# fallenshock/SinDDM

Hardware: AMD Instinct MI355X
Metric: diffusion steps/sec (finest scale) + imgs/sec full multi-scale sample, 1/2/4/8 GPU (higher is better)
Workload: dtype f32 (3x3 convs: binary16 hi/lo split products -- Winograd-domain GEMMs with all 4 MFMA terms, fp32 accumulate; fp32-equivalent, error vs float64 = the fp32 oracle's: tests/test_gpu_h2.py; everything else fp32); 1 GPU; C3: 6-scale pyramid, T=1000, finest scale 411x512, batch 64 per GPU, dim=160; batch_per_gpu=64, global_batch=64, scale=5, parallelism=independent chains over 1 GPU(s), one all-gather of the images

## Files before the change

### sinddm_amd/csrc/conv_wh.h

```cpp
#pragma once
#include <utility>
#include "split16.h"

namespace sinddm {

template <class F, int... I>
__device__ __forceinline__ void wh_static_for_impl(F&& f, std::integer_sequence<int, I...>) {
    (f(std::integral_constant<int, I>{}), ...);
}
template <int N, class F>
__device__ __forceinline__ void wh_static_for(F&& f) {
    wh_static_for_impl(f, std::make_integer_sequence<int, N>{});
}

#ifndef WH_ABL
#define WH_ABL 0
#endif
#ifndef WH_MIXLO
#define WH_MIXLO 1
#endif
#ifndef WH_NT
#define WH_NT 6
#endif
#ifdef WH_TIMING
__device__ unsigned long long g_wh_seg[8 * 256 * 8 * 32];
#define WH_SEG(slot) do { if (j == 2) g_wh_seg[((p.mtp * 256 + blockIdx.x) * 8 + wv) * 32 + (slot)] = __builtin_amdgcn_s_memtime(); } while (0)
#else
#define WH_SEG(slot) do {} while (0)
#endif
constexpr int WH_TH = 8, WH_TW = 32;
constexpr int WH_RS = 40;
constexpr int WH_PS = 408;
constexpr int WH_RAW = 16 * WH_PS * 4;
constexpr int WH_V = 24 * 2 * 64 * 16;
constexpr int WH_XS = 36;
constexpr int WH_X = 2 * 6 * 32 * WH_XS * 4;
constexpr int WH_LDS = 160 * 1024;
constexpr int WH_REGION = WH_LDS - WH_RAW;
constexpr int WH_VB = WH_REGION - WH_V;
static_assert(WH_X <= WH_VB && WH_V + WH_X <= WH_REGION && WH_VB % 16 == 0, "exchange buffer beside either V buffer");
constexpr int WH_TARGET_EXP = 10;
constexpr int WH_COB = 80;

inline bool wh_shape_ok(int cin, int cout) { return cin >= 32 && cin % 16 == 0 && cout % WH_COB == 0; }
inline long long wh_image_halfs(int cin, int cout) { return (long long)(cout / WH_COB) * (cin / 16) * 24 * 5 * 512; }

__device__ __forceinline__ int wh_shift_for(float m, int target) {
    const unsigned bits = __float_as_uint(m) & 0x7fffffffu;
    const int e = (int)(bits >> 23);
    if (e == 0 || e == 255) return 0;
    int s = target - (e - 127);
    return s > 100 ? 100 : (s < -100 ? -100 : s);
}

__device__ __forceinline__ void wh_u24(const float* __restrict__ w, long long base, int transpose, double (&u)[24]) {
    const double G2[4][3] = {{1., 0., 0.}, {.5, .5, .5}, {.5, -.5, .5}, {0., 0., 1.}};
    const double G4[6][3] = {{1. / 4, 0., 0.}, {-1. / 6, -1. / 6, -1. / 6}, {-1. / 6, 1. / 6, -1. / 6},
                             {1. / 24, 1. / 12, 1. / 6}, {1. / 24, -1. / 12, 1. / 6}, {0., 0., 1.}};
    double g[3][3];
#pragma unroll
    for (int a = 0; a < 3; ++a)
#pragma unroll
        for (int b = 0; b < 3; ++b) g[a][b] = (double)(transpose ? w[base + (2 - a) * 3 + (2 - b)] : w[base + a * 3 + b]);
#pragma unroll
    for (int i = 0; i < 4; ++i)
#pragma unroll
        for (int j = 0; j < 6; ++j) {
            double acc = 0.;
#pragma unroll
            for (int a = 0; a < 3; ++a) {
                double r = 0.;
#pragma unroll
                for (int b = 0; b < 3; ++b) r += G4[j][b] * g[a][b];
                acc += G2[i][a] * r;
            }
            u[i * 6 + j] = acc;
        }
}

__global__ __launch_bounds__(256) void wh_wscale_kernel(const float* __restrict__ w, float* __restrict__ wsinv, int cin,
                                                         int cout, int transpose) {
    const int m = blockIdx.x;
    const int M = transpose ? cin : cout, K = transpose ? cout : cin;
    float mx = 0.f;
    if (m < M)
        for (int k = threadIdx.x; k < K; k += 256) {
            double u[24];
            wh_u24(w, transpose ? ((long long)k * cin + m) * 9 : ((long long)m * cin + k) * 9, transpose, u);
#pragma unroll
            for (int f = 0; f < 24; ++f) mx = fmaxf(mx, fabsf((float)u[f]));
        }
    __shared__ float red[4];
#pragma unroll
    for (int o = 32; o > 0; o >>= 1) mx = fmaxf(mx, __shfl_xor(mx, o));
    if ((threadIdx.x & 63) == 0) red[threadIdx.x >> 6] = mx;
    __syncthreads();
    if (threadIdx.x == 0 && m < M) {
        mx = fmaxf(fmaxf(red[0], red[1]), fmaxf(red[2], red[3]));
        wsinv[m] = h2_pow2(-h2_shift_for(mx));
    }
}

__global__ __launch_bounds__(256) void wh_pack_kernel(const float* __restrict__ w, const float* __restrict__ wsinv,
                                                       _Float16* __restrict__ img, int cin, int cout, int transpose,
                                                       long long total) {
    const long long i = (long long)blockIdx.x * 256 + threadIdx.x;
    if (i >= total) return;
    const int M = transpose ? cin : cout, K = transpose ? cout : cin;
    const int nch = K / 16;
    long long r = i;
    const int e = (int)(r % 8); r /= 8;
    const int co16 = (int)(r % 16); r /= 16;
    const int kh = (int)(r % 2); r /= 2;
    const int n = (int)(r % 5); r /= 5;
    const int ch = (int)(r % nch); r /= nch;
    const int cb = (int)r;
    const int m = cb * WH_COB + n * 16 + co16;
    const int k = ch * 16 + kh * 8 + e;
    double u[24];
    if (m < M && k < K) wh_u24(w, transpose ? ((long long)k * cin + m) * 9 : ((long long)m * cin + k) * 9, transpose, u);
    else {
#pragma unroll
        for (int f = 0; f < 24; ++f) u[f] = 0.;
    }
    const double sc = m < M ? 1.0 / (double)wsinv[m] : 1.0;
#pragma unroll
    for (int f = 0; f < 24; ++f) {
        const double s = u[f] * sc;
        const _Float16 hi = (_Float16)(float)s;
        const _Float16 lo = (_Float16)(float)(s - (double)(float)hi);
        const long long o = ((((long long)(cb * nch + ch) * 24 + f) * 5 + n) * 2) * 256 + (kh * 16 + co16) * 8 + e;
        img[o] = hi;
        img[o + 256] = lo;
    }
}

inline int wh_pack_launch(const float* w, float* wsinv, void* img, int cin, int cout, int transpose, hipStream_t st) {
    const int M = transpose ? cin : cout, K = transpose ? cout : cin;
    hipLaunchKernelGGL(wh_wscale_kernel, dim3(M), dim3(256), 0, st, w, wsinv, cin, cout, transpose);
    SINDDM_LAUNCH_CHECK();
    const long long total = (long long)(M / WH_COB) * (K / 16) * 5 * 2 * 16 * 8;
    hipLaunchKernelGGL(wh_pack_kernel, dim3((unsigned)((total + 255) / 256)), dim3(256), 0, st, w, wsinv,
                       static_cast<_Float16*>(img), cin, cout, transpose, total);
    SINDDM_LAUNCH_CHECK();
    return 0;
}

__device__ __forceinline__ void wh_barrier() { asm volatile("s_waitcnt lgkmcnt(0)\n\ts_barrier" ::: "memory"); }

__device__ __forceinline__ float wh_dpp_shr2(float old, float src) {
    return __builtin_bit_cast(float, __builtin_amdgcn_update_dpp(__builtin_bit_cast(int, old), __builtin_bit_cast(int, src), 0x112, 0xf, 0xf, false));
}
__device__ __forceinline__ float wh_dpp_shl2(float old, float src) {
    return __builtin_bit_cast(float, __builtin_amdgcn_update_dpp(__builtin_bit_cast(int, old), __builtin_bit_cast(int, src), 0x102, 0xf, 0xf, false));
}

__global__ __launch_bounds__(512) void conv_wh_kernel(ConvArgs p, int items_per_xcd, int wg_per_xcd) {
    typedef __attribute__((address_space(3))) float lds_f;
    extern __shared__ __attribute__((aligned(16))) float smem[];
    unsigned char* const sbytes = reinterpret_cast<unsigned char*>(smem);
    unsigned char* const sRaw = sbytes;
    unsigned char* const sV = sbytes + WH_RAW;
    const unsigned lds0 = (unsigned)(size_t)(lds_f*)smem;

    const int tid = threadIdx.x;
    const int lane = tid & 63;
    const int wv = __builtin_amdgcn_readfirstlane(tid >> 6);
    const int l16 = lane & 15, kq = lane >> 4;
    const int H = p.H, W = p.W;
    const int HW = H * W;
    const int Wt = p.Wt > 0 ? p.Wt : W;
    const int nch = p.nch3;
    const bool big_out = __builtin_amdgcn_readfirstlane((size_t)p.B * p.Cout * HW > ((size_t)1 << 28)) != 0;
    constexpr int OOB = 0x40000000;
    const bool service_rt = wv >= 6;
    const int sv = wv - 6;

    const int t_q = lane & 1, t_tc = (lane >> 1) & 7, t_mg = (lane >> 4) & 1, t_trl = lane >> 5;
    const int t_tr = t_mg * 2 + t_trl, t_t16 = t_trl * 8 + t_tc;
    const int t_rdB = (((sv & 1) * 8 + 4 * t_q) * WH_PS + 2 * t_tr * WH_RS + 4 * t_tc + 4) * 4;
    const int t_rdE = (((sv & 1) * 8 + 4 * t_q) * WH_PS + 2 * t_tr * WH_RS + (t_tc == 7 ? 36 : 3)) * 4;
    const int t_wr0 = ((t_mg * 64 + (sv & 1) * 16 + t_t16) * 16) + t_q * 8;
    const int fj = service_rt ? 0 : wv;
    const int a_rd = ((kq & 1) * 16 + l16) * 16;

    const int xcd = blockIdx.x & 7, ls = blockIdx.x >> 3;
    const int tpi = p.tilesX * p.tilesY;
    struct Item { int b, y0, x0, cb; bool ok; };
    auto decode = [&](int j) {
        Item it;
        const int li = ls + j * wg_per_xcd;
        const int tl = li / p.coblks;
        it.cb = li - tl * p.coblks;
        const int tile = xcd * p.tiles_per_xcd + tl;
        it.ok = li < items_per_xcd && tile < p.ntiles;
        const int tcl = it.ok ? tile : 0;
        it.b = tcl / tpi;
        const int trm = tcl - it.b * tpi;
        const int tyi = trm / p.tilesX;
        it.y0 = tyi * WH_TH;
        it.x0 = (trm - tyi * p.tilesX) * WH_TW;
        return it;
    };
    auto stage_offsets = [&](const Item& it, int (&vo)[2]) {
#pragma unroll
        for (int ps = 0; ps < 2; ++ps) {
            const int qd = ps * 64 + lane;
            const int r = qd / 10, g = qd - r * 10;
            const int gy = it.y0 - 1 + r, gx = it.x0 - 4 + 4 * g;
            vo[ps] = (qd < 100 && gy >= 0 && gy < H && gx >= 0 && gx < W) ? (gy * W + gx) * 4 : OOB;
        }
    };
    auto role_body = [&](auto ROLE) {
    constexpr bool service = decltype(ROLE)::value;
    f32x4 stg[16];
    auto stage_load = [&](const __amdgpu_buffer_rsrc_t& rs, const int (&vo)[2], int c) {
#pragma unroll
        for (int k = 0; k < 8; ++k) {
            const int so = (c * 16 + (sv & 1) * 8 + k) * HW * 4;
            stg[2 * k] = (WH_ABL & 1) ? f32x4{0.f, 0.f, 0.f, 0.f} : __builtin_bit_cast(f32x4, __builtin_amdgcn_raw_buffer_load_b128(rs, vo[0], so, (WH_NT & 1) ? 2 : 0));
            stg[2 * k + 1] = (WH_ABL & 1) ? f32x4{0.f, 0.f, 0.f, 0.f} : __builtin_bit_cast(f32x4, __builtin_amdgcn_raw_buffer_load_b128(rs, vo[1], so, (WH_NT & 1) ? 2 : 0));
        }
    };
    auto stage_write = [&](unsigned char* raw) {
        unsigned char* dst = raw + (sv & 1) * 8 * WH_PS * 4 + lane * 16;
#pragma unroll
        for (int k = 0; k < 8; ++k) {
            *reinterpret_cast<f32x4*>(dst + k * WH_PS * 4) = stg[2 * k];
            if (lane < 36) *reinterpret_cast<f32x4*>(dst + k * WH_PS * 4 + 1024) = stg[2 * k + 1];
        }
    };
    auto in_rsrc = [&](int b) {
        return __builtin_amdgcn_make_buffer_rsrc(const_cast<float*>(p.in + (size_t)b * p.Cin * HW), 0, p.Cin * HW * 4, 0x00020000);
    };

    Item cur = decode(0);
    if (!cur.ok) return;
    int svoff[2] = {OOB, OOB};
#ifndef WH_SVC_PRIO
#define WH_SVC_PRIO 2
#endif
    if constexpr (service) __builtin_amdgcn_s_setprio(WH_SVC_PRIO);
    if constexpr (service) {
        stage_offsets(cur, svoff);
        stage_load(in_rsrc(cur.b), svoff, 0);
    }
    auto item_scale = [&](const Item& it, float& sxo, float& inv) {
        const int xs = p.amax_in ? wh_shift_for(p.amax_in[(size_t)it.b * AMAX_STRIDE], WH_TARGET_EXP) : 0;
        const float sg = (((it.x0 >> 5) + (it.y0 >> 3) + it.b) & 1) ? -1.0f : 1.0f;
        sxo = sg * h2_pow2(xs);
        inv = sg * h2_pow2(-xs);
    };
    int g = 0;
    auto vbuf = [&](int k) { return sV + ((k & 1) ? WH_VB : 0); };
    for (int j = 0;; ++j) {
        const Item nxt = decode(j + 1);
        const int cb = cur.cb, b = cur.b, y0 = cur.y0, x0 = cur.x0;
        float sx, inv_sx;
        item_scale(cur, sx, inv_sx);

        const __amdgpu_buffer_rsrc_t rsin = in_rsrc(b);

        auto transform = [&](const unsigned char* raw, unsigned char* vb, float sxv) {
            if (WH_ABL & 2) return;
            const f32x2 sx2{sxv, sxv};
            const unsigned char* rpB = raw + t_rdB;
            const unsigned char* rpE = raw + t_rdE;
            unsigned char* wp = vb + t_wr0;
            f32x2 d[2][4][6];
#pragma unroll
            for (int pr = 0; pr < 2; ++pr)
#pragma unroll
                for (int rr = 0; rr < 4; ++rr) {
                    const int o = ((2 * pr) * WH_PS + rr * WH_RS) * 4;
                    const f32x4 a4 = *reinterpret_cast<const f32x4*>(rpB + o), b4 = *reinterpret_cast<const f32x4*>(rpB + o + WH_PS * 4);
                    const float ae = *reinterpret_cast<const float*>(rpE + o), be = *reinterpret_cast<const float*>(rpE + o + WH_PS * 4);
                    d[pr][rr][0] = f32x2{wh_dpp_shr2(ae, a4[3]), wh_dpp_shr2(be, b4[3])};
                    d[pr][rr][1] = f32x2{a4[0], b4[0]}; d[pr][rr][2] = f32x2{a4[1], b4[1]};
                    d[pr][rr][3] = f32x2{a4[2], b4[2]}; d[pr][rr][4] = f32x2{a4[3], b4[3]};
                    d[pr][rr][5] = f32x2{wh_dpp_shl2(ae, a4[0]), wh_dpp_shl2(be, b4[0])};
                }
            wh_static_for<4>([&](auto II) {
                constexpr int i = decltype(II)::value;
                h16x2 hi[2][6], lo[2][6];
#pragma unroll
                for (int pr = 0; pr < 2; ++pr) {
                    f32x2 r[6];
#pragma unroll
                    for (int c = 0; c < 6; ++c)
                        r[c] = i == 0 ? d[pr][0][c] - d[pr][2][c] : i == 1 ? d[pr][1][c] + d[pr][2][c]
                             : i == 2 ? d[pr][2][c] - d[pr][1][c] : d[pr][1][c] - d[pr][3][c];
                    const f32x2 s24 = r[4] - 4.f * r[2], s13 = r[3] - 4.f * r[1];
                    const f32x2 u24 = r[4] - r[2], d31 = r[3] - r[1];
                    f32x2 v[6];
                    v[0] = 4.f * r[0] + (r[4] - 5.f * r[2]);
                    v[1] = s24 + s13;
                    v[2] = s24 - s13;
                    v[3] = u24 + 2.f * d31;
                    v[4] = u24 - 2.f * d31;
                    v[5] = 4.f * r[1] + (r[5] - 5.f * r[3]);
#pragma unroll
                    for (int j = 0; j < 6; ++j) {
                        const f32x2 sc = v[j] * sx2;
                        hi[pr][j] = __builtin_convertvector(sc, h16x2);
#if WH_MIXLO
                        lo[pr][j] = h16x2{(_Float16)__builtin_fmaf(v[j].x, sxv, -(float)hi[pr][j].x), (_Float16)__builtin_fmaf(v[j].y, sxv, -(float)hi[pr][j].y)};
#else
                        const f32x2 rem{__builtin_fmaf(v[j].x, sxv, -(float)hi[pr][j].x), __builtin_fmaf(v[j].y, sxv, -(float)hi[pr][j].y)};
                        lo[pr][j] = __builtin_convertvector(rem, h16x2);
#endif
                    }
                }
#pragma unroll
                for (int j = 0; j < 6; ++j) {
                    using h16x4 = __attribute__((ext_vector_type(4))) _Float16;
                    *reinterpret_cast<h16x4*>(wp + (i * 6 + j) * 2048) = h16x4{hi[0][j][0], hi[0][j][1], hi[1][j][0], hi[1][j][1]};
                    *reinterpret_cast<h16x4*>(wp + (i * 6 + j) * 2048 + 512) = h16x4{lo[0][j][0], lo[0][j][1], lo[1][j][0], lo[1][j][1]};
                }
            });
        };

        f32x4 acc[4][2][5];
#pragma unroll
        for (int a = 0; a < 4; ++a)
#pragma unroll
            for (int g = 0; g < 2; ++g)
#pragma unroll
                for (int n = 0; n < 5; ++n) acc[a][g][n] = f32x4{0.f, 0.f, 0.f, 0.f};
        const __amdgpu_buffer_rsrc_t rsw =
            __builtin_amdgcn_make_buffer_rsrc(const_cast<float*>(p.w3), 0, 0x7FFFFFF0, 0x00020000);
        const int wlane = lane * 16;
        const int wbase = ((cb * nch) * 24 + fj) * 5 * 1024;
        h16x8 ur[10];
        auto load_u = [&](int c, int fi, int n, int slot) {
            const int so = wbase + (c * 24 * 5 + fi * 30 + n) * 1024;
            ur[slot] = __builtin_bit_cast(h16x8, __builtin_amdgcn_raw_buffer_load_b128(rsw, wlane, so, 0));
        };
        auto multiply = [&](int c, const unsigned char* vb) {
            const unsigned char* A = vb + fj * 2048 + a_rd;
            wh_static_for<4>([&](auto FI) {
                constexpr int fi = decltype(FI)::value;
                constexpr int fo = fi * 6 * 2048;
                h16x8 ah0, ah1, al0, al1;
                ah0 = *reinterpret_cast<const h16x8*>(A + fo);
                ah1 = *reinterpret_cast<const h16x8*>(A + fo + 1024);
                al0 = *reinterpret_cast<const h16x8*>(A + fo + 512);
                al1 = *reinterpret_cast<const h16x8*>(A + fo + 1024 + 512);
                wh_static_for<5>([&](auto NN) {
                    constexpr int n = decltype(NN)::value;
                    constexpr int slot = (fi & 1) * 5 + n;
                    const h16x8 u = ur[slot];
                    __builtin_amdgcn_sched_barrier(0);
                    if (WH_ABL & 8) {
                        asm volatile("" ::"v"(ah0), "v"(ah1), "v"(al0), "v"(al1), "v"(u));
                    } else {
                        acc[fi][0][n] = __builtin_amdgcn_mfma_f32_16x16x32_f16(al0, u, acc[fi][0][n], 0, 0, 0);
                        acc[fi][1][n] = __builtin_amdgcn_mfma_f32_16x16x32_f16(al1, u, acc[fi][1][n], 0, 0, 0);
                        acc[fi][0][n] = __builtin_amdgcn_mfma_f32_16x16x32_f16(ah0, u, acc[fi][0][n], 0, 0, 0);
                        acc[fi][1][n] = __builtin_amdgcn_mfma_f32_16x16x32_f16(ah1, u, acc[fi][1][n], 0, 0, 0);
                    }
                    __builtin_amdgcn_sched_barrier(0);
                    if (!(WH_ABL & 4)) {
                        if (fi < 2) load_u(c, fi + 2, n, slot);
                        else load_u(c + 1 < nch ? c + 1 : c, fi - 2, n, slot);
                    }
                    __builtin_amdgcn_sched_barrier(0);
                });
            });
        };

        const int e_t = tid & 31, e_co = tid >> 5;
        const int e_tr = e_t >> 3, e_tc = e_t & 7;
        const int ey = y0 + 2 * e_tr, ex = x0 + 4 * e_tc;
        f32x4 rsd[5][2];
        float ek[5], ebv[5];
        auto ep_operands = [&]() {
            const bool e_in = ex < W;
#pragma unroll
            for (int n = 0; n < 5; ++n) {
                const int co = cb * WH_COB + n * 16 + e_co;
                ek[n] = inv_sx * p.wsinv[co];
                ebv[n] = p.bias ? p.bias[co] : 0.0f;
#pragma unroll
                for (int pp = 0; pp < 2; ++pp) {
                    rsd[n][pp] = f32x4{0.f, 0.f, 0.f, 0.f};
                    if (p.resid && !(WH_ABL & 16) && e_in && ey + pp < H)
                        rsd[n][pp] = ((WH_NT & 2) && big_out) ? __builtin_nontemporal_load(reinterpret_cast<const f32x4*>(p.resid + ((size_t)b * p.Cout + co) * HW + (size_t)(ey + pp) * W + ex))
                                                 : *reinterpret_cast<const f32x4*>(p.resid + ((size_t)b * p.Cout + co) * HW + (size_t)(ey + pp) * W + ex);
                }
            }
        };

        WH_SEG(0);
        if constexpr (service) {
            const __amdgpu_buffer_rsrc_t rsnx = in_rsrc(nxt.ok ? nxt.b : b);
            float sxn = 0.f, inv_n = 0.f;
            if (nxt.ok) item_scale(nxt, sxn, inv_n);
            if (j == 0) {
                stage_write(sRaw);
                if (nch > 1) stage_load(rsin, svoff, 1);
                else if (nxt.ok) { stage_offsets(nxt, svoff); stage_load(rsnx, svoff, 0); }
                WH_SEG(1);
                transform(sRaw, vbuf(g), sx);
                wh_barrier();
            }
            WH_SEG(2);
            for (int c = 0; c < nch; ++c) {
                if (c + 1 < nch || nxt.ok) {
                    stage_write(sRaw);
                    if (c + 2 < nch) stage_load(rsin, svoff, c + 2);
                    else if (nxt.ok) {
                        if (c + 2 == nch) stage_offsets(nxt, svoff);
                        if (c + 2 == nch || nch > 1) stage_load(rsnx, svoff, c + 2 - nch);
                    }
                    if (c == 3) WH_SEG(24);
                    transform(sRaw, vbuf(g + c + 1), c + 1 < nch ? sx : sxn);
                    if (c == 3) WH_SEG(25);
                }
                wh_barrier();
                if (c < 12) WH_SEG(3 + c);
            }
            ep_operands();
        } else {
            wh_static_for<10>([&](auto SL) {
                constexpr int sl = decltype(SL)::value;
                load_u(0, sl / 5, sl % 5, sl);
            });
            WH_SEG(1);
            if (j == 0) wh_barrier();
            WH_SEG(2);
            for (int c = 0; c < nch; ++c) {
                multiply(c, vbuf(g + c));
                if (c == 3) WH_SEG(25);
                wh_barrier();
                if (c < 12) WH_SEG(3 + c);
            }
            ep_operands();
        }
        g += nch;
        WH_SEG(16);

        const int e_wr = ((fj * 32 + l16) * WH_XS + 4 * kq) * 4;
        const int e_rd = (e_co * WH_XS + e_t) * 4;
        float amax = 0.f;
        WH_SEG(17);
        if constexpr (!service) {
#pragma unroll
            for (int mg = 0; mg < 2; ++mg)
#pragma unroll
                for (int n = 0; n < 5; ++n) {
                    acc[0][mg][n] = acc[0][mg][n] + acc[1][mg][n] + acc[2][mg][n];
                    acc[1][mg][n] = acc[1][mg][n] - acc[2][mg][n] - acc[3][mg][n];
                }
        }
        wh_static_for<3>([&](auto PS) {
            constexpr int n0 = 2 * decltype(PS)::value;
            constexpr int nn = n0 + 2 <= 5 ? 2 : 1;
            unsigned char* X = sV + ((g & 1) ? 0 : WH_V);
            if constexpr (!service) {
#pragma unroll
                for (int r = 0; r < 2; ++r)
#pragma unroll
                    for (int nl = 0; nl < nn; ++nl)
#pragma unroll
                        for (int mg = 0; mg < 2; ++mg)
                            *reinterpret_cast<f32x4*>(X + e_wr + (r * 6 * 32 + nl * 16) * (WH_XS * 4) + mg * 64) = acc[r][mg][n0 + nl];
            }
            wh_barrier();
            WH_SEG(18 + decltype(PS)::value);
            float q[nn][2][6];
#pragma unroll
            for (int nl = 0; nl < nn; ++nl)
#pragma unroll
                for (int r = 0; r < 2; ++r)
#pragma unroll
                    for (int j = 0; j < 6; ++j)
                        q[nl][r][j] = *reinterpret_cast<const float*>(X + e_rd + ((r * 6 + j) * 32 + nl * 16) * (WH_XS * 4));
            wh_barrier();
            wh_static_for<nn>([&](auto NL) {
                constexpr int n = n0 + decltype(NL)::value;
                const int co = cb * WH_COB + n * 16 + e_co;
                const float k = ek[n];
                const float bv = ebv[n];
#pragma unroll
                for (int pp = 0; pp < 2; ++pp) {
                    const float* z = q[decltype(NL)::value][pp];
                    const float s12 = z[1] + z[2], d12 = z[1] - z[2], s34 = z[3] + z[4], d34 = z[3] - z[4];
                    f32x4 v{z[0] + s12 + s34, d12 + 2.f * d34, s12 + 4.f * s34, d12 + 8.f * d34 + z[5]};
                    const int y = ey + pp;
                    if ((WH_ABL & 16) && v[0] != 123.456f) continue;
                    if (y < H && ex < W) {
                        const size_t o = ((size_t)b * p.Cout + co) * HW + (size_t)y * W + ex;
                        v = v * k + bv;
                        if (p.out_pre) *reinterpret_cast<f32x4*>(p.out_pre + o) = v;
                        if (p.act == 1) v = gelu_erf4(v);
                        else if (p.act == 2) {
                            const f32x4 a = *reinterpret_cast<const f32x4*>(p.aux + o);
#pragma unroll
                            for (int e = 0; e < 4; ++e) v[e] *= gelu_erf_grad(a[e]);
                        }
                        v += rsd[n][pp];
                        if (ex + 4 > Wt) {
#pragma unroll
                            for (int e = 0; e < 4; ++e) v[e] = ex + e < Wt ? v[e] : 0.0f;
                        }
#pragma unroll
                        for (int e = 0; e < 4; ++e) amax = fmaxf(amax, fabsf(v[e]));
                        if ((WH_NT & 4) && big_out) __builtin_nontemporal_store(v, reinterpret_cast<f32x4*>(p.out + o));
                        else *reinterpret_cast<f32x4*>(p.out + o) = v;
                    }
                }
            });
        });
        if (p.amax_out) amax_publish(amax, p.amax_out + (size_t)b * AMAX_STRIDE);
        WH_SEG(23);
        if (!nxt.ok) break;
        cur = nxt;
    }
    };
    if (service_rt) role_body(std::true_type{});
    else role_body(std::false_type{});
}

#ifndef SINDDM_WH_MIN_ITEMS_PER_CU
#define SINDDM_WH_MIN_ITEMS_PER_CU 12
#endif
#ifndef SINDDM_WH_MIN_PIXELS
#define SINDDM_WH_MIN_PIXELS 12000
#endif
#ifndef SINDDM_CONV_WH
#define SINDDM_CONV_WH 1
#endif
inline bool conv_wh_applies(bool fp32_convs, int B, int H, int W, int cin, int cout) {
    if (!SINDDM_CONV_WH || fp32_convs || !wh_shape_ok(cin, cout) || W % 4 != 0) return false;
    if ((long long)cin * H * W * 4 >= 0x40000000LL) return false;
    if ((long long)H * W < SINDDM_WH_MIN_PIXELS) return false;
    return (long long)B * ((W + WH_TW - 1) / WH_TW) * ((H + WH_TH - 1) / WH_TH) * (cout / WH_COB) >=
           (long long)SINDDM_WH_MIN_ITEMS_PER_CU * wino2_cu_count();
}

inline int conv_wh_launch(const ConvArgs& a_in, hipStream_t st) {
    ConvArgs a = a_in;
    if (!wh_shape_ok(a.Cin, a.Cout) || a.W % 4 != 0 || !a.wsinv || (long long)a.Cin * a.H * a.W * 4 >= 0x40000000LL)
        return SINDDM_E_BADSHAPE;
    ConvProfiler& prof = conv_profiler();
    const bool rec = prof.on && prof.used < ConvProfiler::MAXREC;
    if (rec) {
        while (prof.created <= prof.used) {
            (void)hipEventCreate(&prof.ev[2 * prof.created]);
            (void)hipEventCreate(&prof.ev[2 * prof.created + 1]);
            ++prof.created;
        }
        (void)hipEventRecord(prof.ev[2 * prof.used], st);
    }
    a.nch3 = a.Cin / 16;
    a.coblks = a.Cout / WH_COB;
    a.tilesX = (a.W + WH_TW - 1) / WH_TW;
    a.tilesY = (a.H + WH_TH - 1) / WH_TH;
    a.ntiles = a.B * a.tilesX * a.tilesY;
    a.tiles_per_xcd = (a.ntiles + 7) / 8;
    const int ipx = a.tiles_per_xcd * a.coblks;
    int wpx = wino2_cu_count() / 8;
    if (wpx < 1) wpx = 1;
    if (wpx > ipx) wpx = ipx;
    static const hipError_t attr_rc = hipFuncSetAttribute(reinterpret_cast<const void*>(&conv_wh_kernel),
                                                          hipFuncAttributeMaxDynamicSharedMemorySize, WH_LDS);
    if (attr_rc != hipSuccess) return (int)attr_rc;
#ifdef WH_TIMING
    static int wh_launch_no = 0;
    a.mtp = wh_launch_no++ % 8;
#endif
    hipLaunchKernelGGL(conv_wh_kernel, dim3(wpx * 8), dim3(512), WH_LDS, st, a, ipx, wpx);
    if (rec) {
        (void)hipEventRecord(prof.ev[2 * prof.used + 1], st);
        const double fl = 2.0 * a.B * a.H * (a.Wt > 0 ? a.Wt : a.W) * (double)a.Cout * 9.0 * a.Cin;
        prof.note(1, fl, 2.0 * a.ntiles * 32.0 * 24.0 * 4.0 * (double)a.Cout * a.Cin, 8);
    }
    SINDDM_LAUNCH_CHECK();
    return 0;
}

}
```

### sinddm_amd/csrc/plan.h

```cpp
#pragma once
#include <stdint.h>

namespace sinddm {

constexpr int KC = 8;
constexpr int TIME_DIM = 32;
constexpr int CHANNELS = 3;

inline bool wh_plan_ok(int cin, int cout) { return cin >= 32 && cin % 16 == 0 && cout % 80 == 0; }
inline long long wh_plan_halfs(int cin, int cout) { return (long long)(cout / 80) * (cin / 16) * 24 * 5 * 512; }

struct BlockPlan {
    int cin, cout;
    int64_t mlp_w, mlp_b, tr_w, tr_b, dw_w, dw_b, c1_w, c1_b, c2_w, c2_b, res_w, res_b;
    int mt;
    int coblks;
    int co_lds;
    int nch1;
    int nch2;
    int nchr;
    int64_t pk_c1, pk_c2, pk_res, pk_b1, pk_b2;
    int nchw1, nchw2;
    int64_t pk_wc1, pk_wc2;
    int64_t pk_w1f, pk_w2f;
    int64_t pk_q1, pk_q2, pk_qs1, pk_qs2;
    int cond_off;
};

struct NetPlan {
    int dim, half;
    BlockPlan blk[4];
    int64_t tm0_w, tm0_b, tm2_w, tm2_b, fin_w, fin_b;
    int64_t nparams, npacked;
    int64_t pk_zero;
    int ntensors;
    int64_t tensor_off[64];
    int cond_stride;
    bool fp32_convs;
    bool ok;
};

inline int mt_for(int cout) { return (cout % 80 == 0) ? 5 : ((cout % 32 == 0) ? 2 : 1); }
inline int co_lds_for(int mt) { int m = mt * 16; return (m % 32 == 16) ? m : m + 16; }

inline NetPlan make_plan(int dim_arg) {
    NetPlan p{};
    const int dim = dim_arg & 0xFFFF;
    p.fp32_convs = (dim_arg & 0x10000) != 0;
    if (dim_arg < 0 || (dim_arg >> 17) != 0) { p.ok = false; return p; }
    p.ok = dim >= 2 && dim % 2 == 0 && dim <= 1024;
    p.dim = dim;
    p.half = dim / 2;
    int64_t o = 0;
    int nt = 0;
    auto take = [&](int64_t n) { int64_t r = o; p.tensor_off[nt++] = r; o += n; return r; };
    p.tm0_w = take(TIME_DIM * 4 * TIME_DIM * 2);
    p.tm0_b = take(TIME_DIM * 4);
    p.tm2_w = take(TIME_DIM * TIME_DIM * 4);
    p.tm2_b = take(TIME_DIM);
    const int cins[4] = {CHANNELS, p.half, dim, dim};
    const int couts[4] = {p.half, dim, dim, p.half};
    int64_t q = 0;
    int coff = 0;
    for (int l = 0; l < 4; ++l) {
        BlockPlan& b = p.blk[l];
        b.cin = cins[l];
        b.cout = couts[l];
        b.mlp_w = take(TIME_DIM * TIME_DIM);
        b.mlp_b = take(TIME_DIM);
        b.tr_w = take((int64_t)b.cin * TIME_DIM);
        b.tr_b = take(b.cin);
        b.dw_w = take((int64_t)b.cin * 25);
        b.dw_b = take(b.cin);
        b.c1_w = take((int64_t)b.cout * b.cin * 9);
        b.c1_b = take(b.cout);
        b.c2_w = take((int64_t)b.cout * b.cout * 9);
        b.c2_b = take(b.cout);
        if (b.cin != b.cout) {
            b.res_w = take((int64_t)b.cout * b.cin);
            b.res_b = take(b.cout);
        } else {
            b.res_w = b.res_b = -1;
        }
        b.mt = mt_for(b.cout);
        b.coblks = (b.cout + b.mt * 16 - 1) / (b.mt * 16);
        b.co_lds = co_lds_for(b.mt);
        b.nch1 = (b.cin + KC - 1) / KC;
        b.nch2 = (b.cout + KC - 1) / KC;
        b.nchr = (b.res_w >= 0) ? (b.cin + KC - 1) / KC : 0;
        b.pk_c1 = q; q += (int64_t)b.coblks * b.nch1 * 9 * KC * b.co_lds;
        b.pk_c2 = q; q += (int64_t)b.coblks * b.nch2 * 9 * KC * b.co_lds;
        b.pk_res = q; q += (int64_t)b.coblks * b.nchr * KC * b.co_lds;
        b.pk_b1 = q; q += (int64_t)b.coblks * b.mt * 16;
        b.pk_b2 = q; q += (int64_t)b.coblks * b.mt * 16;
        b.nchw1 = (b.cin + 15) / 16;
        b.nchw2 = (b.cout + 15) / 16;
        if (b.cin >= 8) { b.pk_wc1 = q; q += (int64_t)b.coblks * b.nchw1 * 16 * 4 * b.mt * 64; } else b.pk_wc1 = -1;
        b.pk_wc2 = q; q += (int64_t)b.coblks * b.nchw2 * 16 * 4 * b.mt * 64;
        const bool f24 = b.mt == 5 && b.cout % 80 == 0;
        if (f24 && b.cin >= 16 && b.cin % 16 == 0) { b.pk_w1f = q; q += (int64_t)b.coblks * b.nchw1 * 32768; } else b.pk_w1f = -1;
        if (f24 && b.cout % 16 == 0) { b.pk_w2f = q; q += (int64_t)b.coblks * b.nchw2 * 32768; } else b.pk_w2f = -1;
        q = (q + 63) / 64 * 64;
        if (wh_plan_ok(b.cin, b.cout)) {
            b.pk_q1 = q; q += wh_plan_halfs(b.cin, b.cout) / 2;
            b.pk_qs1 = q; q += (b.cout + 63) / 64 * 64;
        } else b.pk_q1 = b.pk_qs1 = -1;
        if (wh_plan_ok(b.cout, b.cout)) {
            b.pk_q2 = q; q += wh_plan_halfs(b.cout, b.cout) / 2;
            b.pk_qs2 = q; q += (b.cout + 63) / 64 * 64;
        } else b.pk_q2 = b.pk_qs2 = -1;
        b.cond_off = coff;
        coff += b.cin;
    }
    p.fin_w = take((int64_t)CHANNELS * p.half);
    p.fin_b = take(CHANNELS);
    p.nparams = o;
    p.pk_zero = q;
    q += 64;
    p.npacked = q;
    p.ntensors = nt;
    p.cond_stride = (coff + 3) / 4 * 4;
    return p;
}

}
```

Measured before the change: 711.6 sample-steps/s (finest scale, batch x steps/s, all GPUs).

## Prefetch next item's Winograd weights and overlap epilogue stores across items

The Winograd conv kernel now keeps the weight register ring alive across work items, so the last channel chunk prefetches the next item's first weight fragments instead of reloading them from scratch. It also always issues the next-stage input load at j==0 and moves the output-transform accumulator reduction into the compute path. When a residual is present, it defers each pair of output stores by one group so the global residual adds and stores overlap with the next exchange round. Epilogue operand loads are split behind a scheduling barrier. The changes raise register pressure and make the pipeline logic more intricate.

```diff
diff --git a/sinddm_amd/csrc/conv_wh.h b/sinddm_amd/csrc/conv_wh.h
--- a/sinddm_amd/csrc/conv_wh.h
+++ b/sinddm_amd/csrc/conv_wh.h
@@ -40,9 +40,6 @@
 constexpr int WH_VB = WH_REGION - WH_V;
 static_assert(WH_X <= WH_VB && WH_V + WH_X <= WH_REGION && WH_VB % 16 == 0, "exchange buffer beside either V buffer");
 constexpr int WH_TARGET_EXP = 10;
-constexpr int WH_COB = 80;
-
-inline bool wh_shape_ok(int cin, int cout) { return cin >= 32 && cin % 16 == 0 && cout % WH_COB == 0; }
 inline long long wh_image_halfs(int cin, int cout) { return (long long)(cout / WH_COB) * (cin / 16) * 24 * 5 * 512; }
 
 __device__ __forceinline__ int wh_shift_for(float m, int target) {
@@ -253,6 +250,7 @@
     };
     int g = 0;
     auto vbuf = [&](int k) { return sV + ((k & 1) ? WH_VB : 0); };
+    h16x8 ur[10];
     for (int j = 0;; ++j) {
         const Item nxt = decode(j + 1);
         const int cb = cur.cb, b = cur.b, y0 = cur.y0, x0 = cur.x0;
@@ -324,20 +322,22 @@
 #pragma unroll
         for (int a = 0; a < 4; ++a)
 #pragma unroll
-            for (int g = 0; g < 2; ++g)
-#pragma unroll
-                for (int n = 0; n < 5; ++n) acc[a][g][n] = f32x4{0.f, 0.f, 0.f, 0.f};
+            for (int mg = 0; mg < 2; ++mg)
+#pragma unroll
+                for (int n = 0; n < 5; ++n) acc[a][mg][n] = f32x4{0.f, 0.f, 0.f, 0.f};
         const __amdgpu_buffer_rsrc_t rsw =
             __builtin_amdgcn_make_buffer_rsrc(const_cast<float*>(p.w3), 0, 0x7FFFFFF0, 0x00020000);
         const int wlane = lane * 16;
         const int wbase = ((cb * nch) * 24 + fj) * 5 * 1024;
-        h16x8 ur[10];
-        auto load_u = [&](int c, int fi, int n, int slot) {
-            const int so = wbase + (c * 24 * 5 + fi * 30 + n) * 1024;
+        const int wbase_nxt = (((nxt.ok ? nxt.cb : cb) * nch) * 24 + fj) * 5 * 1024;
+        auto load_u = [&](int base, int fi, int n, int slot) {
+            const int so = base + (fi * 30 + n) * 1024;
             ur[slot] = __builtin_bit_cast(h16x8, __builtin_amdgcn_raw_buffer_load_b128(rsw, wlane, so, 0));
         };
         auto multiply = [&](int c, const unsigned char* vb) {
             const unsigned char* A = vb + fj * 2048 + a_rd;
+            const int ubase = wbase + c * (24 * 5 * 1024);
+            const int unext = c + 1 < nch ? ubase + 24 * 5 * 1024 : wbase_nxt;
             wh_static_for<4>([&](auto FI) {
                 constexpr int fi = decltype(FI)::value;
                 constexpr int fo = fi * 6 * 2048;
@@ -361,8 +361,8 @@
                     }
                     __builtin_amdgcn_sched_barrier(0);
                     if (!(WH_ABL & 4)) {
-                        if (fi < 2) load_u(c, fi + 2, n, slot);
-                        else load_u(c + 1 < nch ? c + 1 : c, fi - 2, n, slot);
+                        if (fi < 2) load_u(ubase, fi + 2, n, slot);
+                        else load_u(unext, fi - 2, n, slot);
                     }
                     __builtin_amdgcn_sched_barrier(0);
                 });
@@ -381,6 +381,11 @@
                 const int co = cb * WH_COB + n * 16 + e_co;
                 ek[n] = inv_sx * p.wsinv[co];
                 ebv[n] = p.bias ? p.bias[co] : 0.0f;
+            }
+            __builtin_amdgcn_sched_barrier(0);
+#pragma unroll
+            for (int n = 0; n < 5; ++n) {
+                const int co = cb * WH_COB + n * 16 + e_co;
 #pragma unroll
                 for (int pp = 0; pp < 2; ++pp) {
                     rsd[n][pp] = f32x4{0.f, 0.f, 0.f, 0.f};
@@ -398,8 +403,7 @@
             if (nxt.ok) item_scale(nxt, sxn, inv_n);
             if (j == 0) {
                 stage_write(sRaw);
-                if (nch > 1) stage_load(rsin, svoff, 1);
-                else if (nxt.ok) { stage_offsets(nxt, svoff); stage_load(rsnx, svoff, 0); }
+                stage_load(rsin, svoff, 1);
                 WH_SEG(1);
                 transform(sRaw, vbuf(g), sx);
                 wh_barrier();
@@ -411,7 +415,7 @@
                     if (c + 2 < nch) stage_load(rsin, svoff, c + 2);
                     else if (nxt.ok) {
                         if (c + 2 == nch) stage_offsets(nxt, svoff);
-                        if (c + 2 == nch || nch > 1) stage_load(rsnx, svoff, c + 2 - nch);
+                        stage_load(rsnx, svoff, c + 2 - nch);
                     }
                     if (c == 3) WH_SEG(24);
                     transform(sRaw, vbuf(g + c + 1), c + 1 < nch ? sx : sxn);
@@ -422,10 +426,11 @@
             }
             ep_operands();
         } else {
-            wh_static_for<10>([&](auto SL) {
-                constexpr int sl = decltype(SL)::value;
-                load_u(0, sl / 5, sl % 5, sl);
-            });
+            if (j == 0 || (WH_ABL & 4))
+                wh_static_for<10>([&](auto SL) {
+                    constexpr int sl = decltype(SL)::value;
+                    load_u(wbase, sl / 5, sl % 5, sl);
+                });
             WH_SEG(1);
             if (j == 0) wh_barrier();
             WH_SEG(2);
@@ -435,6 +440,14 @@
                 wh_barrier();
                 if (c < 12) WH_SEG(3 + c);
             }
+#pragma unroll
+            for (int mg = 0; mg < 2; ++mg)
+#pragma unroll
+                for (int n = 0; n < 5; ++n) {
+                    acc[0][mg][n] = acc[0][mg][n] + acc[1][mg][n] + acc[2][mg][n];
+                    acc[1][mg][n] = acc[1][mg][n] - acc[2][mg][n] - acc[3][mg][n];
+                    asm volatile("" : "+v"(acc[0][mg][n]), "+v"(acc[1][mg][n]) :: "memory");
+                }
             ep_operands();
         }
         g += nch;
@@ -443,16 +456,27 @@
         const int e_wr = ((fj * 32 + l16) * WH_XS + 4 * kq) * 4;
         const int e_rd = (e_co * WH_XS + e_t) * 4;
         float amax = 0.f;
+        const bool defer = p.resid != nullptr;
+        f32x4 kept[2][2];
+#pragma unroll
+        for (int nl = 0; nl < 2; ++nl) kept[nl][0] = kept[nl][1] = f32x4{0.f, 0.f, 0.f, 0.f};
+        auto finish = [&](int n, int pp, f32x4 v) {
+            const int y = ey + pp;
+            if ((WH_ABL & 16) && v[0] != 123.456f) return;
+            if (y < H && ex < W) {
+                const size_t o = ((size_t)b * p.Cout + cb * WH_COB + n * 16 + e_co) * HW + (size_t)y * W + ex;
+                v += rsd[n][pp];
+                if (ex + 4 > Wt) {
+#pragma unroll
+                    for (int e = 0; e < 4; ++e) v[e] = ex + e < Wt ? v[e] : 0.0f;
+                }
+#pragma unroll
+                for (int e = 0; e < 4; ++e) amax = fmaxf(amax, fabsf(v[e]));
+                if ((WH_NT & 4) && big_out) __builtin_nontemporal_store(v, reinterpret_cast<f32x4*>(p.out + o));
+                else *reinterpret_cast<f32x4*>(p.out + o) = v;
+            }
+        };
         WH_SEG(17);
-        if constexpr (!service) {
-#pragma unroll
-            for (int mg = 0; mg < 2; ++mg)
-#pragma unroll
-                for (int n = 0; n < 5; ++n) {
-                    acc[0][mg][n] = acc[0][mg][n] + acc[1][mg][n] + acc[2][mg][n];
-                    acc[1][mg][n] = acc[1][mg][n] - acc[2][mg][n] - acc[3][mg][n];
-                }
-        }
         wh_static_for<3>([&](auto PS) {
             constexpr int n0 = 2 * decltype(PS)::value;
             constexpr int nn = n0 + 2 <= 5 ? 2 : 1;
@@ -477,18 +501,18 @@
                     for (int j = 0; j < 6; ++j)
                         q[nl][r][j] = *reinterpret_cast<const float*>(X + e_rd + ((r * 6 + j) * 32 + nl * 16) * (WH_XS * 4));
             wh_barrier();
+            f32x4 vf[nn][2];
             wh_static_for<nn>([&](auto NL) {
-                constexpr int n = n0 + decltype(NL)::value;
+                constexpr int nl = decltype(NL)::value, n = n0 + nl;
                 const int co = cb * WH_COB + n * 16 + e_co;
                 const float k = ek[n];
                 const float bv = ebv[n];
 #pragma unroll
                 for (int pp = 0; pp < 2; ++pp) {
-                    const float* z = q[decltype(NL)::value][pp];
+                    const float* z = q[nl][pp];
                     const float s12 = z[1] + z[2], d12 = z[1] - z[2], s34 = z[3] + z[4], d34 = z[3] - z[4];
                     f32x4 v{z[0] + s12 + s34, d12 + 2.f * d34, s12 + 4.f * s34, d12 + 8.f * d34 + z[5]};
                     const int y = ey + pp;
-                    if ((WH_ABL & 16) && v[0] != 123.456f) continue;
                     if (y < H && ex < W) {
                         const size_t o = ((size_t)b * p.Cout + co) * HW + (size_t)y * W + ex;
                         v = v * k + bv;
@@ -499,19 +523,29 @@
 #pragma unroll
                             for (int e = 0; e < 4; ++e) v[e] *= gelu_erf_grad(a[e]);
                         }
-                        v += rsd[n][pp];
-                        if (ex + 4 > Wt) {
-#pragma unroll
-                            for (int e = 0; e < 4; ++e) v[e] = ex + e < Wt ? v[e] : 0.0f;
-                        }
-#pragma unroll
-                        for (int e = 0; e < 4; ++e) amax = fmaxf(amax, fabsf(v[e]));
-                        if ((WH_NT & 4) && big_out) __builtin_nontemporal_store(v, reinterpret_cast<f32x4*>(p.out + o));
-                        else *reinterpret_cast<f32x4*>(p.out + o) = v;
                     }
+                    vf[nl][pp] = v;
                 }
             });
+            if (!defer) {
+                wh_static_for<nn>([&](auto NL) {
+                    constexpr int nl = decltype(NL)::value;
+                    finish(n0 + nl, 0, vf[nl][0]);
+                    finish(n0 + nl, 1, vf[nl][1]);
+                });
+            } else {
+                if constexpr (n0 > 0) {
+                    finish(n0 - 2, 0, kept[0][0]); finish(n0 - 2, 1, kept[0][1]);
+                    finish(n0 - 1, 0, kept[1][0]); finish(n0 - 1, 1, kept[1][1]);
+                }
+                wh_static_for<nn>([&](auto NL) {
+                    constexpr int nl = decltype(NL)::value;
+                    kept[nl][0] = vf[nl][0];
+                    kept[nl][1] = vf[nl][1];
+                });
+            }
         });
+        if (defer) { finish(4, 0, kept[0][0]); finish(4, 1, kept[0][1]); }
         if (p.amax_out) amax_publish(amax, p.amax_out + (size_t)b * AMAX_STRIDE);
         WH_SEG(23);
         if (!nxt.ok) break;
diff --git a/sinddm_amd/csrc/plan.h b/sinddm_amd/csrc/plan.h
--- a/sinddm_amd/csrc/plan.h
+++ b/sinddm_amd/csrc/plan.h
@@ -7,8 +7,10 @@
 constexpr int TIME_DIM = 32;
 constexpr int CHANNELS = 3;
 
-inline bool wh_plan_ok(int cin, int cout) { return cin >= 32 && cin % 16 == 0 && cout % 80 == 0; }
-inline long long wh_plan_halfs(int cin, int cout) { return (long long)(cout / 80) * (cin / 16) * 24 * 5 * 512; }
+constexpr int WH_COB = 80;
+inline bool wh_shape_ok(int cin, int cout) { return cin >= 32 && cin % 16 == 0 && cout % WH_COB == 0; }
+inline bool wh_plan_ok(int cin, int cout) { return wh_shape_ok(cin, cout); }
+inline long long wh_plan_halfs(int cin, int cout) { return (long long)(cout / WH_COB) * (cin / 16) * 24 * 5 * 512; }
 
 struct BlockPlan {
     int cin, cout;
```

Measured after the change: 695.1 sample-steps/s (finest scale, batch x steps/s, all GPUs). 0.977x the previous value.
